# SimeonZhang/detectron2_tensorflow

Hardware: AMD Instinct MI355X
Metric: img/sec whole-node Mask R-CNN R50-FPN @1333x800 (higher is better)
Workload: dtype f32

## Files before the change

### detectron2_tensorflow_amd/csrc/conv_wgrad.hip

```cpp
#include "common.h"
#include "conv_plan.h"
#include "internal.h"

namespace d2mi {
namespace {

typedef float floatx16 __attribute__((ext_vector_type(16)));

constexpr int KP = kWgradKP;

struct WgradArgs {
  const float* x;
  const float* dy;
  float* dw;
  float* partial;
  float* dbias;
  float* pbias;
  int N, H, W, Cin, Cout, KH, KW, stride, pad, OH, OW;
  int P;
  int nCi, nCo, ntiles;
  int splits, chunks_per_split, nchunks;
  int part;
  int x_bytes, dy_bytes;
  int prio;
  int xcd;
  const uint32_t* bitmap;
};

__device__ __forceinline__ void wgrad_tile_split(const WgradArgs& a, int& tile, int& split) {
  if (!a.xcd) {
    tile = blockIdx.x;
    split = blockIdx.y;
    return;
  }
  const int nwg = gridDim.x * gridDim.y;
  const int L = blockIdx.x + blockIdx.y * gridDim.x;
  const int q = nwg / 8, r8 = nwg % 8, x8 = L % 8;
  const int l = (x8 < r8 ? x8 * (q + 1) : r8 * (q + 1) + (x8 - r8) * q) + L / 8;
  split = l / gridDim.x;
  tile = l - split * gridDim.x;
}

template <int TM, int TN>
__global__ __launch_bounds__(256, 2) void conv_wgrad_kernel(WgradArgs a) {
  constexpr int BM = 2 * TM * 32, BN = 2 * TN * 32;
  constexpr int PA = BM + 32, PB = BN + 32;
  constexpr int CA = BM / 4, CB = BN / 4;
  constexpr int RA = KP * CA / 256, RB = KP * CB / 256;
  __shared__ __attribute__((aligned(16))) float As[KP * PA];
  __shared__ __attribute__((aligned(16))) float Bs[KP * PB];

  const int tile = blockIdx.x;
  const int per_tap = a.nCi * a.nCo;
  const int tap = tile / per_tap;
  const int rem = tile - tap * per_tap;
  const int cit = rem / a.nCo, cot = rem - cit * a.nCo;
  const int kh = tap / a.KW, kw = tap - kh * a.KW;
  const int ci0 = cit * BM, co0 = cot * BN;
  const int split = blockIdx.y;
  const int c_begin = split * a.chunks_per_split;
  const int c_end = min(a.nchunks, c_begin + a.chunks_per_split);

  const int tid = threadIdx.x;
  const int lane = tid & 63, wave = tid >> 6;
  const int wr = wave >> 1, wc = wave & 1;
  const int li = lane & 31, lh = lane >> 5;

  float4 ra[RA], rb[RB];
  auto load_chunk = [&](int ch) {
    const int pbase = ch * KP;
#pragma unroll
    for (int q = 0; q < RA; ++q) {
      const int idx = tid + 256 * q;
      const int row = idx / CA, c4 = idx - row * CA;
      const int p = pbase + row;
      const int ci = ci0 + c4 * 4;
      float4 v = make_float4(0.f, 0.f, 0.f, 0.f);
      if (p < a.P && ci < a.Cin) {
        const int n = p / (a.OH * a.OW);
        const int r2 = p - n * a.OH * a.OW;
        const int oy = r2 / a.OW, ox = r2 - oy * a.OW;
        const int iy = oy * a.stride - a.pad + kh, ix = ox * a.stride - a.pad + kw;
        if (iy >= 0 && iy < a.H && ix >= 0 && ix < a.W)
          v = *reinterpret_cast<const float4*>(a.x + (((size_t)n * a.H + iy) * a.W + ix) * a.Cin +
                                               ci);
      }
      ra[q] = v;
    }
#pragma unroll
    for (int q = 0; q < RB; ++q) {
      const int idx = tid + 256 * q;
      const int row = idx / CB, c4 = idx - row * CB;
      const int p = pbase + row;
      const int co = co0 + c4 * 4;
      rb[q] = (p < a.P && co < a.Cout)
                  ? *reinterpret_cast<const float4*>(a.dy + (size_t)p * a.Cout + co)
                  : make_float4(0.f, 0.f, 0.f, 0.f);
    }
  };
  auto store_chunk = [&]() {
#pragma unroll
    for (int q = 0; q < RA; ++q) {
      const int idx = tid + 256 * q;
      const int row = idx / CA, c4 = idx - row * CA;
      *reinterpret_cast<float4*>(&As[row * PA + c4 * 4]) = ra[q];
    }
#pragma unroll
    for (int q = 0; q < RB; ++q) {
      const int idx = tid + 256 * q;
      const int row = idx / CB, c4 = idx - row * CB;
      *reinterpret_cast<float4*>(&Bs[row * PB + c4 * 4]) = rb[q];
    }
  };

  floatx16 acc[TM][TN];
#pragma unroll
  for (int i = 0; i < TM; ++i)
#pragma unroll
    for (int j = 0; j < TN; ++j)
#pragma unroll
      for (int r = 0; r < 16; ++r) acc[i][j][r] = 0.f;

  const bool do_bias = a.dbias != nullptr && tap == 0 && cit == 0;
  float bsum = 0.f;

  if (c_begin < c_end) {
    load_chunk(c_begin);
    for (int ch = c_begin; ch < c_end; ++ch) {
      store_chunk();
      __syncthreads();
      if (ch + 1 < c_end) load_chunk(ch + 1);
      if (do_bias && tid < BN) {
#pragma unroll 8
        for (int k = 0; k < KP; ++k) bsum += Bs[k * PB + tid];
      }
#pragma unroll 4
      for (int k = 0; k < KP; k += 2) {
        const float* Ar = &As[(k + lh) * PA + wr * TM * 32 + li];
        const float* Br = &Bs[(k + lh) * PB + wc * TN * 32 + li];
        float fa[TM], fb[TN];
#pragma unroll
        for (int i = 0; i < TM; ++i) fa[i] = Ar[i * 32];
#pragma unroll
        for (int j = 0; j < TN; ++j) fb[j] = Br[j * 32];
#pragma unroll
        for (int i = 0; i < TM; ++i)
#pragma unroll
          for (int j = 0; j < TN; ++j)
            acc[i][j] = __builtin_amdgcn_mfma_f32_32x32x2f32(fa[i], fb[j], acc[i][j], 0, 0, 0);
      }
      __syncthreads();
    }
  }

  if (do_bias && tid < BN && co0 + tid < a.Cout) {
    if (a.part) a.pbias[(size_t)split * a.Cout + co0 + tid] = bsum;
    else a.dbias[co0 + tid] = bsum;
  }

  const size_t wsz = (size_t)a.KH * a.KW * a.Cin * a.Cout;
  float* out = a.part ? a.partial + (size_t)split * wsz : a.dw;
#pragma unroll
  for (int j = 0; j < TN; ++j) {
    const int co = co0 + (wc * TN + j) * 32 + li;
    if (co >= a.Cout) continue;
#pragma unroll
    for (int i = 0; i < TM; ++i) {
      const int cb = ci0 + (wr * TM + i) * 32 + 4 * lh;
#pragma unroll
      for (int r = 0; r < 16; ++r) {
        const int ci = cb + (r & 3) + 8 * (r >> 2);
        if (ci < a.Cin) out[((size_t)tap * a.Cin + ci) * a.Cout + co] = acc[i][j][r];
      }
    }
  }
}

__global__ void wgrad_reduce4_kernel(const float4* __restrict__ partial, int splits, size_t total4,
                                     float4* __restrict__ dw, const float* __restrict__ pbias,
                                     int Cout, float* __restrict__ dbias, int accum) {
  const size_t n = total4 + (dbias ? (size_t)Cout : 0);
  for (size_t i = blockIdx.x * (size_t)blockDim.x + threadIdx.x; i < n;
       i += (size_t)gridDim.x * blockDim.x) {
    if (i < total4) {
      float4 s = make_float4(0.f, 0.f, 0.f, 0.f);
#pragma unroll 4
      for (int k = 0; k < splits; ++k) {
        const float4 v = partial[(size_t)k * total4 + i];
        s.x += v.x;
        s.y += v.y;
        s.z += v.z;
        s.w += v.w;
      }
      if (accum) {
        const float4 o = dw[i];
        s.x = o.x + s.x;
        s.y = o.y + s.y;
        s.z = o.z + s.z;
        s.w = o.w + s.w;
      }
      dw[i] = s;
    } else {
      const size_t c = i - total4;
      float s = 0.f;
#pragma unroll 8
      for (int k = 0; k < splits; ++k) s += pbias[(size_t)k * Cout + c];
      dbias[c] = accum ? dbias[c] + s : s;
    }
  }
}

__global__ void wgrad_reduce_kernel(const float* __restrict__ partial, int splits, size_t total,
                                    float* __restrict__ dw, const float* __restrict__ pbias,
                                    int Cout, float* __restrict__ dbias, int accum) {
  for (size_t i = blockIdx.x * (size_t)blockDim.x + threadIdx.x; i < total + Cout;
       i += (size_t)gridDim.x * blockDim.x) {
    if (i < total) {
      float s = 0.f;
#pragma unroll 4
      for (int k = 0; k < splits; ++k) s += partial[(size_t)k * total + i];
      dw[i] = accum ? dw[i] + s : s;
    } else if (dbias) {
      const size_t c = i - total;
      float s = 0.f;
#pragma unroll 8
      for (int k = 0; k < splits; ++k) s += pbias[(size_t)k * Cout + c];
      dbias[c] = accum ? dbias[c] + s : s;
    }
  }
}


typedef short bf16x8 __attribute__((ext_vector_type(8)));
constexpr int LDW = 32;

__device__ __forceinline__ int wswz(int row, int elem) {
  return row * LDW + ((((elem >> 3) ^ (row >> 2)) & 3) << 3) + (elem & 7);
}

struct FastDiv {
  uint32_t d, m, l;
};
__device__ __forceinline__ uint32_t fdiv(uint32_t n, const FastDiv& f) {
  return (__umulhi(n, f.m) + n) >> f.l;
}

template <int TM, int TN, int OCC = 2>
__global__ __launch_bounds__(256, OCC) void conv_wgrad_split_kernel(WgradArgs a, FastDiv fd_hw,
                                                                    FastDiv fd_w) {
  constexpr int BM = 2 * TM * 32, BN = 2 * TN * 32;
  constexpr int GA = BM / 4, GB = BN / 4;
  __shared__ __attribute__((aligned(16))) uint16_t As[3 * BM * LDW];
  __shared__ __attribute__((aligned(16))) uint16_t Bs[3 * BN * LDW];
  __shared__ float bred[8][BN];

  int tile, split;
  wgrad_tile_split(a, tile, split);
  const int per_tap = a.nCi * a.nCo;
  const int tap = tile / per_tap;
  const int rem = tile - tap * per_tap;
  const int cit = rem / a.nCo, cot = rem - cit * a.nCo;
  const int kh = tap / a.KW, kw = tap - kh * a.KW;
  const int ci0 = cit * BM, co0 = cot * BN;
  const int c_begin = split * a.chunks_per_split;
  const int c_end = min(a.nchunks, c_begin + a.chunks_per_split);

  const int tid = threadIdx.x;
  const int lane = tid & 63, wave = tid >> 6;
  const int wr = wave >> 1, wc = wave & 1;
  const int li = lane & 31, lh = lane >> 5;

  const bool a_on = tid < 8 * GA, b_on = tid < 8 * GB;
  const int cga = tid % GA, pga = tid / GA;
  const int cgb = tid % GB, pgb = tid / GB;
  const int ci = ci0 + 4 * cga, co = co0 + 4 * cgb;
  const bool ci_ok = a_on && ci < a.Cin, co_ok = b_on && co < a.Cout;

  const __amdgpu_buffer_rsrc_t xr = __builtin_amdgcn_make_buffer_rsrc(
      const_cast<float*>(a.x), 0, a.x_bytes, 0x00020000);
  const __amdgpu_buffer_rsrc_t yr = __builtin_amdgcn_make_buffer_rsrc(
      const_cast<float*>(a.dy), 0, a.dy_bytes, 0x00020000);
  constexpr uint32_t kOOB = 0x80000000u;

  float4 ra[4], rb[4];
  auto load_chunk = [&](int ch) {
#pragma unroll
    for (int q = 0; q < 4; ++q) {
      const int p = ch * KP + 4 * pga + q;
      const uint32_t n = fdiv((uint32_t)p, fd_hw);
      const int r2 = p - (int)n * (a.OH * a.OW);
      const int oy = (int)fdiv((uint32_t)r2, fd_w), ox = r2 - oy * a.OW;
      const int iy = oy * a.stride - a.pad + kh, ix = ox * a.stride - a.pad + kw;
      const bool ok = ci_ok & (p < a.P) & ((unsigned)iy < (unsigned)a.H) &
                      ((unsigned)ix < (unsigned)a.W);
      const uint32_t off = ok ? (uint32_t)(((((int)n * a.H + iy) * a.W + ix) * a.Cin + ci) * 4) : kOOB;
      ra[q] = __builtin_bit_cast(float4, __builtin_amdgcn_raw_buffer_load_b128(xr, off, 0, 0));
      const int pb = ch * KP + 4 * pgb + q;
      const uint32_t offb = (co_ok & (pb < a.P)) ? (uint32_t)((pb * a.Cout + co) * 4) : kOOB;
      rb[q] = __builtin_bit_cast(float4, __builtin_amdgcn_raw_buffer_load_b128(yr, offb, 0, 0));
    }
  };
  const bool do_bias = a.dbias != nullptr && tap == 0 && cit == 0;
  float bsum[4] = {0.f, 0.f, 0.f, 0.f};
  auto store_chunk = [&]() {
    if (a_on) {
      const float* f = reinterpret_cast<const float*>(ra);
#pragma unroll
      for (int j = 0; j < 4; ++j) {
        uint2 h, m, l;
        split3(make_float4(f[j], f[4 + j], f[8 + j], f[12 + j]), h, m, l);
        const int o = wswz(4 * cga + j, 4 * pga);
        *reinterpret_cast<uint2*>(&As[o]) = h;
        *reinterpret_cast<uint2*>(&As[BM * LDW + o]) = m;
        *reinterpret_cast<uint2*>(&As[2 * BM * LDW + o]) = l;
      }
    }
    if (b_on) {
      const float* f = reinterpret_cast<const float*>(rb);
#pragma unroll
      for (int j = 0; j < 4; ++j) {
        const float4 v = make_float4(f[j], f[4 + j], f[8 + j], f[12 + j]);
        if (do_bias) bsum[j] += ((v.x + v.y) + v.z) + v.w;
        uint2 h, m, l;
        split3(v, h, m, l);
        const int o = wswz(4 * cgb + j, 4 * pgb);
        *reinterpret_cast<uint2*>(&Bs[o]) = h;
        *reinterpret_cast<uint2*>(&Bs[BN * LDW + o]) = m;
        *reinterpret_cast<uint2*>(&Bs[2 * BN * LDW + o]) = l;
      }
    }
  };

  floatx16 acc[TM][TN];
#pragma unroll
  for (int i = 0; i < TM; ++i)
#pragma unroll
    for (int j = 0; j < TN; ++j)
#pragma unroll
      for (int r = 0; r < 16; ++r) acc[i][j][r] = 0.f;

  if (c_begin < c_end) {
    load_chunk(c_begin);
    for (int ch = c_begin; ch < c_end; ++ch) {
      store_chunk();
      __syncthreads();
      if (ch + 1 < c_end) load_chunk(ch + 1);
      if (a.prio) __builtin_amdgcn_s_setprio(1);
#pragma unroll
      for (int ks = 0; ks < 2; ++ks) {
        bf16x8 fa[3][TM], fb[3][TN];
#pragma unroll
        for (int pl = 0; pl < 3; ++pl) {
#pragma unroll
          for (int i = 0; i < TM; ++i)
            fa[pl][i] = *reinterpret_cast<const bf16x8*>(
                &As[pl * BM * LDW + wswz((wr * TM + i) * 32 + li, ks * 16 + lh * 8)]);
#pragma unroll
          for (int j = 0; j < TN; ++j)
            fb[pl][j] = *reinterpret_cast<const bf16x8*>(
                &Bs[pl * BN * LDW + wswz((wc * TN + j) * 32 + li, ks * 16 + lh * 8)]);
        }
        constexpr int PAi[6] = {1, 2, 0, 0, 1, 0};
        constexpr int PBi[6] = {1, 0, 2, 1, 0, 0};
#pragma unroll
        for (int t = 0; t < 6; ++t)
#pragma unroll
          for (int i = 0; i < TM; ++i)
#pragma unroll
            for (int j = 0; j < TN; ++j)
              acc[i][j] = __builtin_amdgcn_mfma_f32_32x32x16_bf16(fa[PAi[t]][i], fb[PBi[t]][j],
                                                                   acc[i][j], 0, 0, 0);
      }
      if (a.prio) __builtin_amdgcn_s_setprio(0);
      __syncthreads();
    }
  }

  if (do_bias) {
    if (b_on) {
#pragma unroll
      for (int j = 0; j < 4; ++j) bred[pgb][4 * cgb + j] = bsum[j];
    }
    __syncthreads();
    if (tid < BN && co0 + tid < a.Cout) {
      float s = 0.f;
#pragma unroll
      for (int g = 0; g < 8; ++g) s += bred[g][tid];
      if (a.part) a.pbias[(size_t)split * a.Cout + co0 + tid] = s;
      else a.dbias[co0 + tid] = s;
    }
  }

  const size_t wsz = (size_t)a.KH * a.KW * a.Cin * a.Cout;
  float* out = a.part ? a.partial + (size_t)split * wsz : a.dw;
#pragma unroll
  for (int j = 0; j < TN; ++j) {
    const int oc = co0 + (wc * TN + j) * 32 + li;
    if (oc >= a.Cout) continue;
#pragma unroll
    for (int i = 0; i < TM; ++i) {
      const int cb = ci0 + (wr * TM + i) * 32 + 4 * lh;
#pragma unroll
      for (int r = 0; r < 16; ++r) {
        const int c = cb + (r & 3) + 8 * (r >> 2);
        if (c < a.Cin) out[((size_t)tap * a.Cin + c) * a.Cout + oc] = acc[i][j][r];
      }
    }
  }
}


template <int LD, bool INC = false, bool LIST = false>
__global__ __launch_bounds__(1024, 1) void conv_wgrad_ws_kernel(WgradArgs a, FastDiv fd_hw,
                                                                FastDiv fd_w) {
  static_assert(!(LIST && INC), "the listed chunks are not consecutive");
  constexpr int TM = 2, TN = 2, BM = 256, BN = 128, S = 2;
  constexpr int GA = BM / 4, GB = BN / 4;
  constexpr int A_H = 3 * BM * LDW, B_H = 3 * BN * LDW;
  constexpr int STAGE = A_H + B_H;
  __shared__ __attribute__((aligned(16))) uint16_t smem[S * STAGE];
  __shared__ float bred[8][BN];
  __shared__ uint16_t clist[LIST ? kWgradListCap : 1];
  __shared__ int wcnt[LIST ? 17 : 1];

  int tile, split;
  wgrad_tile_split(a, tile, split);
  const int per_tap = a.nCi * a.nCo;
  const int tap = tile / per_tap;
  const int rem = tile - tap * per_tap;
  const int cit = rem / a.nCo, cot = rem - cit * a.nCo;
  const int kh = tap / a.KW, kw = tap - kh * a.KW;
  const int ci0 = cit * BM, co0 = cot * BN;
  const int c_begin = split * a.chunks_per_split;
  const int c_end = min(a.nchunks, c_begin + a.chunks_per_split);

  const int tid = threadIdx.x;
  const int lane = tid & 63;
  const int wave = __builtin_amdgcn_readfirstlane(tid >> 6);
  int nks = max(c_end - c_begin, 0);
  if constexpr (LIST) {
    const int nall = nks;
    int base = 0;
    for (int i0 = 0; i0 < nall; i0 += 1024) {
      const int i = i0 + tid;
      bool set = false;
      if (i < nall) {
        const int ch = c_begin + i;
        set = (a.bitmap[ch >> 5] >> (ch & 31)) & 1u;
      }
      const unsigned long long b = __ballot(set);
      if (lane == 0) wcnt[wave] = __popcll(b);
      __syncthreads();
      int before = base;
      for (int w = 0; w < 16; ++w) {
        const int c = wcnt[w];
        before += w < wave ? c : 0;
        base += c;
      }
      if (set) clist[before + __popcll(b & ((1ull << lane) - 1ull))] = (uint16_t)i;
      __syncthreads();
    }
    nks = __builtin_amdgcn_readfirstlane(base);
  }
  const int wr = wave >> 1, wc = wave & 1;
  const int li = lane & 31, lh = lane >> 5;
  const bool do_bias = a.dbias != nullptr && tap == 0 && cit == 0;

  floatx16 acc[TM][TN];
#pragma unroll
  for (int i = 0; i < TM; ++i)
#pragma unroll
    for (int j = 0; j < TN; ++j)
#pragma unroll
      for (int r = 0; r < 16; ++r) acc[i][j][r] = 0.f;

  if (wave >= 8) {
    const int st = tid - 512;
    const int cga = st % GA, pga = st / GA;
    const bool b_on = st >= 256;
    const int sb = st - 256;
    const int cgb = (b_on ? sb : 0) % GB, pgb = (b_on ? sb : 0) / GB;
    const int ci = ci0 + 4 * cga, co = co0 + 4 * cgb;
    const bool ci_ok = ci < a.Cin, co_ok = b_on && co < a.Cout;
    const __amdgpu_buffer_rsrc_t xr = __builtin_amdgcn_make_buffer_rsrc(
        const_cast<float*>(a.x), 0, a.x_bytes, 0x00020000);
    const __amdgpu_buffer_rsrc_t yr = __builtin_amdgcn_make_buffer_rsrc(
        const_cast<float*>(a.dy), 0, a.dy_bytes, 0x00020000);
    constexpr uint32_t kOOB = 0x80000000u;
    float4 ra[LD][4], rb[LD][4];
    const int clast = c_begin + max(nks, 1) - 1;
    int c_ch = c_begin;
    const int jlast = max(nks, 1) - 1;
    int j_ld = 0;
    const int c_first = (LIST && nks > 0) ? c_begin + clist[0] : c_begin;
    int p0 = c_first * KP + 4 * pga;
    int pb0 = c_first * KP + 4 * pgb;
    int oy0 = 0, ox0 = 0;
    if (INC) {
      const int r2 = p0 - (int)fdiv((uint32_t)p0, fd_hw) * (a.OH * a.OW);
      oy0 = (int)fdiv((uint32_t)r2, fd_w);
      ox0 = r2 - oy0 * a.OW;
    }
    const int dy32 = KP / a.OW, dx32 = KP - (KP / a.OW) * a.OW;
    const int ybase = kh - a.pad, xbase = kw - a.pad;
    const int tsh = ybase * a.W + xbase;
    const uint32_t bstride = (uint32_t)KP * (uint32_t)a.Cout * 4u;
    uint32_t boff = (uint32_t)(pb0 * a.Cout + co) * 4u;
    auto load = [&](float4 (&la)[4], float4 (&lb)[4]) {
#pragma unroll
      for (int q = 0; q < 4; ++q) {
        const int p = p0 + q;
        uint32_t off;
        if (INC) {
          int ox = ox0 + q, oy = oy0;
          const bool wrap = ox >= a.OW;
          ox = wrap ? ox - a.OW : ox;
          oy = wrap ? oy + 1 : oy;
          oy = oy >= a.OH ? oy - a.OH : oy;
          const bool ok = ci_ok & (p < a.P) & ((unsigned)(oy + ybase) < (unsigned)a.H) &
                          ((unsigned)(ox + xbase) < (unsigned)a.W);
          off = ok ? (__umul24((uint32_t)(p + tsh), (uint32_t)a.Cin) + (uint32_t)ci) * 4u : kOOB;
        } else {
          const int n = (int)fdiv((uint32_t)p, fd_hw);
          const int r2 = p - n * (a.OH * a.OW);
          const int oy = (int)fdiv((uint32_t)r2, fd_w), ox = r2 - oy * a.OW;
          const int iy = oy * a.stride - a.pad + kh, ix = ox * a.stride - a.pad + kw;
          const bool ok = ci_ok & (p < a.P) & ((unsigned)iy < (unsigned)a.H) &
                          ((unsigned)ix < (unsigned)a.W);
          off = ok ? (uint32_t)(((((int)n * a.H + iy) * a.W + ix) * a.Cin + ci) * 4) : kOOB;
        }
        la[q] = __builtin_bit_cast(float4, __builtin_amdgcn_raw_buffer_load_b128(xr, off, 0, 0));
        const uint32_t offb = (co_ok & (pb0 + q < a.P)) ? boff + (uint32_t)(q * a.Cout * 4) : kOOB;
        lb[q] = __builtin_bit_cast(float4, __builtin_amdgcn_raw_buffer_load_b128(yr, offb, 0, 0));
      }
      if constexpr (LIST) {
        if (j_ld < jlast) {
          ++j_ld;
          const int ch = c_begin + clist[j_ld];
          p0 = ch * KP + 4 * pga;
          pb0 = ch * KP + 4 * pgb;
          boff = (uint32_t)(pb0 * a.Cout + co) * 4u;
        }
      } else if (c_ch < clast) {
        ++c_ch;
        p0 += KP;
        pb0 += KP;
        boff += bstride;
        if (INC) {
          ox0 += dx32;
          oy0 += dy32;
          const bool wrap = ox0 >= a.OW;
          ox0 = wrap ? ox0 - a.OW : ox0;
          oy0 = wrap ? oy0 + 1 : oy0;
          oy0 = oy0 >= a.OH ? oy0 - a.OH : oy0;
        }
      }
    };
    float bsum[4] = {0.f, 0.f, 0.f, 0.f};
    auto write = [&](int buf, const float4 (&la)[4], const float4 (&lb)[4]) {
      uint16_t* As = smem + buf * STAGE;
      uint16_t* Bs = As + A_H;
      const float* f = reinterpret_cast<const float*>(la);
#pragma unroll
      for (int j = 0; j < 4; ++j) {
        uint2 h, m, l;
        split3(make_float4(f[j], f[4 + j], f[8 + j], f[12 + j]), h, m, l);
        const int o = wswz(4 * cga + j, 4 * pga);
        *reinterpret_cast<uint2*>(&As[o]) = h;
        *reinterpret_cast<uint2*>(&As[BM * LDW + o]) = m;
        *reinterpret_cast<uint2*>(&As[2 * BM * LDW + o]) = l;
      }
      if (b_on) {
        const float* g = reinterpret_cast<const float*>(lb);
#pragma unroll
        for (int j = 0; j < 4; ++j) {
          const float4 v = make_float4(g[j], g[4 + j], g[8 + j], g[12 + j]);
          if (do_bias) bsum[j] += ((v.x + v.y) + v.z) + v.w;
          uint2 h, m, l;
          split3(v, h, m, l);
          const int o = wswz(4 * cgb + j, 4 * pgb);
          *reinterpret_cast<uint2*>(&Bs[o]) = h;
          *reinterpret_cast<uint2*>(&Bs[BN * LDW + o]) = m;
          *reinterpret_cast<uint2*>(&Bs[2 * BN * LDW + o]) = l;
        }
      }
    };
#pragma unroll
    for (int j = 0; j < LD; ++j) load(ra[j], rb[j]);
    if (nks > 0) write(0, ra[0], rb[0]);
    load(ra[0], rb[0]);
    __syncthreads();
    int u0 = 0;
    for (; u0 + LD <= nks; u0 += LD) {
#pragma unroll
      for (int j = 0; j < LD; ++j) {
        const int v = u0 + j + 1;
        const int set = (j + 1) % LD;
        if (v < nks) write(v & 1, ra[set], rb[set]);
        load(ra[set], rb[set]);
        __syncthreads();
      }
    }
#pragma unroll
    for (int j = 0; j < LD - 1; ++j) {
      if (u0 + j < nks) {
        const int v = u0 + j + 1;
        const int set = (j + 1) % LD;
        if (v < nks) write(v & 1, ra[set], rb[set]);
        __syncthreads();
      }
    }
    if (do_bias && b_on) {
#pragma unroll
      for (int j = 0; j < 4; ++j) bred[pgb][4 * cgb + j] = bsum[j];
    }
  } else {
    bf16x8 fa[3][TM], fb[3][TN];
    auto ld1 = [&](const uint16_t* As, const uint16_t* Bs, int pa, int pb, int ks) {
#pragma unroll
      for (int i = 0; i < TM; ++i)
        fa[pa][i] = *reinterpret_cast<const bf16x8*>(
            &As[pa * BM * LDW + wswz((wr * TM + i) * 32 + li, ks * 16 + lh * 8)]);
#pragma unroll
      for (int j = 0; j < TN; ++j)
        fb[pb][j] = *reinterpret_cast<const bf16x8*>(
            &Bs[pb * BN * LDW + wswz((wc * TN + j) * 32 + li, ks * 16 + lh * 8)]);
    };
    auto mm1 = [&](int pa, int pb) {
#pragma unroll
      for (int i = 0; i < TM; ++i)
#pragma unroll
        for (int j = 0; j < TN; ++j)
          acc[i][j] =
              __builtin_amdgcn_mfma_f32_32x32x16_bf16(fa[pa][i], fb[pb][j], acc[i][j], 0, 0, 0);
    };
    auto step16 = [&](const uint16_t* As, const uint16_t* Bs, int ks) {
      ld1(As, Bs, 1, 1, ks);
      __builtin_amdgcn_sched_barrier(0);
      ld1(As, Bs, 2, 0, ks);
      mm1(1, 1);
      __builtin_amdgcn_sched_barrier(0);
      ld1(As, Bs, 0, 2, ks);
      mm1(2, 0);
      __builtin_amdgcn_sched_barrier(0);
      mm1(0, 2);
      mm1(0, 1);
      mm1(1, 0);
      mm1(0, 0);
    };
    __syncthreads();
    for (int u = 0; u < nks; ++u) {
      const uint16_t* As = smem + (u & 1) * STAGE;
      const uint16_t* Bs = As + A_H;
      if (a.prio) __builtin_amdgcn_s_setprio(1);
      step16(As, Bs, 0);
      step16(As, Bs, 1);
      if (a.prio) __builtin_amdgcn_s_setprio(0);
      __builtin_amdgcn_sched_barrier(0);
      __syncthreads();
    }
  }
  if (do_bias) {
    __syncthreads();
    if (tid < BN && co0 + tid < a.Cout) {
      float s = 0.f;
#pragma unroll
      for (int g = 0; g < 8; ++g) s += bred[g][tid];
      if (a.part) a.pbias[(size_t)split * a.Cout + co0 + tid] = s;
      else a.dbias[co0 + tid] = s;
    }
  }
  if (wave >= 8) return;
  const size_t wsz = (size_t)a.KH * a.KW * a.Cin * a.Cout;
  float* out = a.part ? a.partial + (size_t)split * wsz : a.dw;
#pragma unroll
  for (int j = 0; j < TN; ++j) {
    const int oc = co0 + (wc * TN + j) * 32 + li;
    if (oc >= a.Cout) continue;
#pragma unroll
    for (int i = 0; i < TM; ++i) {
      const int cb = ci0 + (wr * TM + i) * 32 + 4 * lh;
#pragma unroll
      for (int r = 0; r < 16; ++r) {
        const int c = cb + (r & 3) + 8 * (r >> 2);
        if (c < a.Cin) out[((size_t)tap * a.Cin + c) * a.Cout + oc] = acc[i][j][r];
      }
    }
  }
}

FastDiv make_fastdiv(uint32_t d) {
  FastDiv f;
  f.d = d;
  uint32_t l = 0;
  while ((1ull << l) < d) ++l;
  f.l = l;
  f.m = (uint32_t)((((1ull << 32) * ((1ull << l) - d)) / d) + 1);
  return f;
}

}
}

using namespace d2mi;

extern "C" size_t d2mi_conv2d_wgrad_workspace_size(int N, int H, int W, int Cin, int Cout, int KH,
                                                   int KW, int stride, int pad_beg, int pad_end) {
  if (N <= 0 || H <= 0 || W <= 0 || Cin <= 0 || Cout <= 0 || KH <= 0 || KW <= 0 || stride <= 0)
    return 0;
  const ConvShape s = {N, H, W, Cin, Cout, KH, KW, stride, pad_beg, pad_end};
  WgradPlan split, f32;
  if (plan_wgrad(s, kPlanSplit3, kOpAllAligned | kOpWorkspace, SIZE_MAX, &split) ||
      plan_wgrad(s, 0, kOpAllAligned | kOpWorkspace, SIZE_MAX, &f32))
    return 0;
  return std::max(split.ws_bytes, f32.ws_bytes);
}

static int wgrad_plan_checked(int N, int H, int W, int Cin, int Cout, int KH, int KW, int stride,
                              int pad_beg, int pad_end, int flags, int operands,
                              size_t workspace_bytes, WgradPlan* p) {
  D2MI_REQUIRE((flags & ~12) == 0,
               "wgrad flags: bit2 = split-bf16 products, bit3 = accumulate into dw / dbias");
  D2MI_REQUIRE(N > 0 && H > 0 && W > 0 && Cin > 0 && Cout > 0 && KH > 0 && KW > 0 && stride > 0,
               "bad conv shape");
  D2MI_REQUIRE(Cin % 4 == 0 && Cout % 4 == 0, "Cin and Cout must be multiples of 4 (%d, %d)",
               Cin, Cout);
  int OH, OW;
  D2MI_REQUIRE(conv_dims(H, W, KH, KW, stride, pad_beg, pad_end, OH, OW) == 0,
               "conv output is empty");
  D2MI_REQUIRE((long long)N * OH * OW < (1LL << 31), "too many pixels");
  if (flags & kPlanSplit3)
    D2MI_REQUIRE((int64_t)N * H * W * Cin * 4 < (1ll << 31) &&
                     (int64_t)N * OH * OW * Cout * 4 < (1ll << 31),
                 "split wgrad: x and dy must each be < 2 GiB");
  plan_wgrad({N, H, W, Cin, Cout, KH, KW, stride, pad_beg, pad_end}, flags, operands,
             workspace_bytes, p);
  if (flags & kPlanAccum)
    D2MI_REQUIRE((operands & kOpWorkspace) && workspace_bytes >= p->ws_bytes,
                 "accumulating wgrad: workspace must hold %d slab(s)", p->splits);
  return 0;
}

extern "C" int d2mi_conv2d_wgrad_plan(int N, int H, int W, int Cin, int Cout, int KH, int KW,
                                      int stride, int pad_beg, int pad_end, int flags,
                                      int operands, size_t workspace_bytes, int32_t* out,
                                      int out_len) {
  D2MI_REQUIRE((operands & ~127) == 0, "wgrad plan: unknown operand bits");
  WgradPlan p;
  if (wgrad_plan_checked(N, H, W, Cin, Cout, KH, KW, stride, pad_beg, pad_end, flags, operands,
                         workspace_bytes, &p))
    return -1;
  const int32_t v[] = {p.kernel, p.TM, p.TN, p.BM, p.BN, p.nCi, p.nCo, p.ntiles, p.nchunks,
                       p.splits, p.chunks_per_split, p.part, p.reduce, p.reduce_grid,
                       (int32_t)(p.ws_bytes & 0x7fffffff), (int32_t)(p.ws_bytes >> 31)};
  return emit_plan(v, (int)(sizeof(v) / sizeof(v[0])), out, out_len);
}

static int wgrad_launch(const float* x, const float* dy, float* dw_hwio, float* dbias, int N,
                        int H, int W, int Cin, int Cout, int KH, int KW, int stride, int pad_beg,
                        int pad_end, int flags, const uint32_t* bitmap, void* workspace,
                        size_t workspace_bytes, void* stream) {
  auto al16 = [](const void* q) { return ((uintptr_t)q & 15) == 0; };
  WgradPlan p;
  if (wgrad_plan_checked(N, H, W, Cin, Cout, KH, KW, stride, pad_beg, pad_end, flags,
                         (al16(dw_hwio) ? kOpAligned : 0) | (workspace ? kOpWorkspace : 0) |
                             (al16(workspace) ? kOpWsAligned : 0),
                         workspace_bytes, &p))
    return -1;
  D2MI_REQUIRE(al16(x) && al16(dy), "x and dy must be 16-byte aligned");
  WgradSpace sp = {};
  if (p.part) {
    Workspace carve(workspace, workspace_bytes);
    sp.lay(carve, p.splits, (size_t)KH * KW * Cin * Cout, Cout);
  }
  WgradArgs a = {};
  a.prio = tuning(kTuneWgradPrio);
  a.xcd = tuning(kTuneWgradXCD) > 0 ? 1 : 0;
  a.x = x;
  a.dy = dy;
  a.dw = dw_hwio;
  a.dbias = dbias;
  a.N = N;
  a.H = H;
  a.W = W;
  a.Cin = Cin;
  a.Cout = Cout;
  a.KH = KH;
  a.KW = KW;
  a.stride = stride;
  a.pad = pad_beg;
  a.OH = p.OH;
  a.OW = p.OW;
  a.P = N * a.OH * a.OW;
  a.nCi = p.nCi;
  a.nCo = p.nCo;
  a.ntiles = p.ntiles;
  a.splits = p.splits;
  a.chunks_per_split = p.chunks_per_split;
  a.nchunks = p.nchunks;
  a.part = p.part;
  a.partial = sp.dw;
  a.pbias = sp.dbias;
  hipStream_t st = as_stream(stream);
  const dim3 grid(p.ntiles, p.splits);
  if (p.kernel != kWgradF32) {
    a.x_bytes = (int)((int64_t)N * H * W * Cin * 4);
    a.dy_bytes = (int)((int64_t)a.P * Cout * 4);
  }
  const FastDiv fhw = make_fastdiv((uint32_t)(a.OH * a.OW)), fw = make_fastdiv((uint32_t)a.OW);
  const int tm = p.TM, tn = p.TN;
  const bool listed = bitmap != nullptr && p.chunks_per_split <= kWgradListCap &&
                      (p.kernel == kWgradWSInc || p.kernel == kWgradWS);
  a.bitmap = listed ? bitmap : nullptr;
  if (listed)
    hipLaunchKernelGGL((conv_wgrad_ws_kernel<1, false, true>), grid, dim3(1024), 0, st, a, fhw, fw);
  else if (p.kernel == kWgradWSInc)
    hipLaunchKernelGGL((conv_wgrad_ws_kernel<1, true>), grid, dim3(1024), 0, st, a, fhw, fw);
  else if (p.kernel == kWgradWS)
    hipLaunchKernelGGL((conv_wgrad_ws_kernel<1>), grid, dim3(1024), 0, st, a, fhw, fw);
  else if (p.kernel == kWgradSplitOcc3)
    hipLaunchKernelGGL((conv_wgrad_split_kernel<2, 2, 3>), grid, dim3(256), 0, st, a, fhw, fw);
  else if (p.kernel == kWgradSplit && tm == 2 && tn == 2)
    hipLaunchKernelGGL((conv_wgrad_split_kernel<2, 2>), grid, dim3(256), 0, st, a, fhw, fw);
  else if (p.kernel == kWgradSplit && tm == 2)
    hipLaunchKernelGGL((conv_wgrad_split_kernel<2, 1>), grid, dim3(256), 0, st, a, fhw, fw);
  else if (p.kernel == kWgradSplit && tn == 2)
    hipLaunchKernelGGL((conv_wgrad_split_kernel<1, 2>), grid, dim3(256), 0, st, a, fhw, fw);
  else if (p.kernel == kWgradSplit)
    hipLaunchKernelGGL((conv_wgrad_split_kernel<1, 1>), grid, dim3(256), 0, st, a, fhw, fw);
  else if (tm == 2 && tn == 2)
    hipLaunchKernelGGL((conv_wgrad_kernel<2, 2>), grid, dim3(256), 0, st, a);
  else if (tm == 2)
    hipLaunchKernelGGL((conv_wgrad_kernel<2, 1>), grid, dim3(256), 0, st, a);
  else if (tn == 2)
    hipLaunchKernelGGL((conv_wgrad_kernel<1, 2>), grid, dim3(256), 0, st, a);
  else
    hipLaunchKernelGGL((conv_wgrad_kernel<1, 1>), grid, dim3(256), 0, st, a);
  D2MI_LAUNCH_CHECK();
  if (p.reduce == kReduceNone) return listed ? 1 : 0;
  const size_t total = (size_t)KH * KW * Cin * Cout;
  const int accum = (flags & kPlanAccum) != 0;
  if (p.reduce == kReduceFloat4)
    hipLaunchKernelGGL(wgrad_reduce4_kernel, dim3(p.reduce_grid), dim3(256), 0, st,
                       reinterpret_cast<const float4*>(a.partial), a.splits, total / 4,
                       reinterpret_cast<float4*>(dw_hwio), a.pbias, Cout, dbias, accum);
  else
    hipLaunchKernelGGL(wgrad_reduce_kernel, dim3(p.reduce_grid), dim3(256), 0, st, a.partial,
                       a.splits, total, dw_hwio, a.pbias, Cout, dbias, accum);
  D2MI_LAUNCH_CHECK();
  return listed ? 1 : 0;
}

extern "C" int d2mi_conv2d_wgrad_ex(const float* x, const float* dy, float* dw_hwio,
                                    float* dbias, int N, int H, int W, int Cin, int Cout, int KH,
                                    int KW, int stride, int pad_beg, int pad_end, int flags,
                                    void* workspace, size_t workspace_bytes, void* stream) {
  return wgrad_launch(x, dy, dw_hwio, dbias, N, H, W, Cin, Cout, KH, KW, stride, pad_beg, pad_end,
                      flags, nullptr, workspace, workspace_bytes, stream);
}

extern "C" int d2mi_conv2d_wgrad_rows(const float* x, const float* dy, float* dw_hwio,
                                      float* dbias, int N, int H, int W, int Cin, int Cout, int KH,
                                      int KW, int stride, int pad_beg, int pad_end, int flags,
                                      const void* census, size_t census_bytes, void* workspace,
                                      size_t workspace_bytes, void* stream) {
  int OH, OW;
  D2MI_REQUIRE(N > 0 && H > 0 && W > 0 && KH > 0 && KW > 0 && stride > 0 &&
                   conv_dims(H, W, KH, KW, stride, pad_beg, pad_end, OH, OW) == 0 &&
                   (long long)N * OH * OW < (1LL << 31),
               "bad conv shape");
  RowCensusSpace cs;
  Workspace carve(const_cast<void*>(census), census_bytes);
  cs.lay(carve, N * OH * OW, 0);
  D2MI_REQUIRE(census != nullptr && carve.ok(), "row census workspace too small (%zu < %zu)",
               census_bytes, carve.off);
  D2MI_REQUIRE(((uintptr_t)census & 3) == 0, "the row census must be 4-byte aligned");
  return wgrad_launch(x, dy, dw_hwio, dbias, N, H, W, Cin, Cout, KH, KW, stride, pad_beg, pad_end,
                      flags, cs.bitmap, workspace, workspace_bytes, stream);
}


extern "C" int d2mi_conv2d_wgrad(const float* x, const float* dy, float* dw_hwio, float* dbias,
                                 int N, int H, int W, int Cin, int Cout, int KH, int KW,
                                 int stride, int pad_beg, int pad_end, void* workspace,
                                 size_t workspace_bytes, void* stream) {
  return d2mi_conv2d_wgrad_ex(x, dy, dw_hwio, dbias, N, H, W, Cin, Cout, KH, KW, stride,
                              pad_beg, pad_end, 0, workspace, workspace_bytes, stream);
}
```

Measured before the change: 113.2.

## Add two-stage LDS pipeline with deep register prefetch to split wgrad kernel

Adds a variant of the split-K weight-gradient kernel with two LDS stages and a three-chunk register prefetch ring. The bf16 split-and-store and the global loads are interleaved with the MFMA sequence using sched_group_barrier hints, which removes one barrier per chunk. This variant is used only when the grid fits within one wave of CUs (occupancy 1). Larger grids keep the original single-stage kernel. The cost is more LDS and registers per block, plus tail-handling logic that is harder to get right.

```diff
diff --git a/detectron2_tensorflow_amd/csrc/conv_wgrad.hip b/detectron2_tensorflow_amd/csrc/conv_wgrad.hip
--- a/detectron2_tensorflow_amd/csrc/conv_wgrad.hip
+++ b/detectron2_tensorflow_amd/csrc/conv_wgrad.hip
@@ -245,13 +245,15 @@
   return (__umulhi(n, f.m) + n) >> f.l;
 }
 
-template <int TM, int TN, int OCC = 2>
+template <int TM, int TN, int OCC = 2, int LD = 1, int ST = 1>
 __global__ __launch_bounds__(256, OCC) void conv_wgrad_split_kernel(WgradArgs a, FastDiv fd_hw,
                                                                     FastDiv fd_w) {
+  static_assert(ST == 1 || ST == 2, "one or two LDS stages");
   constexpr int BM = 2 * TM * 32, BN = 2 * TN * 32;
   constexpr int GA = BM / 4, GB = BN / 4;
-  __shared__ __attribute__((aligned(16))) uint16_t As[3 * BM * LDW];
-  __shared__ __attribute__((aligned(16))) uint16_t Bs[3 * BN * LDW];
+  constexpr int A_H = 3 * BM * LDW, B_H = 3 * BN * LDW;
+  constexpr int STAGE = A_H + B_H;
+  __shared__ __attribute__((aligned(16))) uint16_t smem[ST * STAGE];
   __shared__ float bred[8][BN];
 
   int tile, split;
@@ -270,7 +272,8 @@
   const int wr = wave >> 1, wc = wave & 1;
   const int li = lane & 31, lh = lane >> 5;
 
-  const bool a_on = tid < 8 * GA, b_on = tid < 8 * GB;
+  const bool a_on = (ST == 2 && 8 * GA >= 256) || tid < 8 * GA;
+  const bool b_on = (ST == 2 && 8 * GB >= 256) || tid < 8 * GB;
   const int cga = tid % GA, pga = tid / GA;
   const int cgb = tid % GB, pgb = tid / GB;
   const int ci = ci0 + 4 * cga, co = co0 + 4 * cgb;
@@ -282,31 +285,34 @@
       const_cast<float*>(a.dy), 0, a.dy_bytes, 0x00020000);
   constexpr uint32_t kOOB = 0x80000000u;
 
-  float4 ra[4], rb[4];
-  auto load_chunk = [&](int ch) {
-#pragma unroll
-    for (int q = 0; q < 4; ++q) {
-      const int p = ch * KP + 4 * pga + q;
-      const uint32_t n = fdiv((uint32_t)p, fd_hw);
-      const int r2 = p - (int)n * (a.OH * a.OW);
-      const int oy = (int)fdiv((uint32_t)r2, fd_w), ox = r2 - oy * a.OW;
-      const int iy = oy * a.stride - a.pad + kh, ix = ox * a.stride - a.pad + kw;
-      const bool ok = ci_ok & (p < a.P) & ((unsigned)iy < (unsigned)a.H) &
-                      ((unsigned)ix < (unsigned)a.W);
-      const uint32_t off = ok ? (uint32_t)(((((int)n * a.H + iy) * a.W + ix) * a.Cin + ci) * 4) : kOOB;
-      ra[q] = __builtin_bit_cast(float4, __builtin_amdgcn_raw_buffer_load_b128(xr, off, 0, 0));
-      const int pb = ch * KP + 4 * pgb + q;
-      const uint32_t offb = (co_ok & (pb < a.P)) ? (uint32_t)((pb * a.Cout + co) * 4) : kOOB;
-      rb[q] = __builtin_bit_cast(float4, __builtin_amdgcn_raw_buffer_load_b128(yr, offb, 0, 0));
-    }
+  float4 ra[LD][4], rb[LD][4];
+  auto load_q = [&](float4 (&la)[4], float4 (&lb)[4], int ch, int q) {
+    const bool in = (LD == 1 && ST == 1) || ch < c_end;
+    const int p = ch * KP + 4 * pga + q;
+    const uint32_t n = fdiv((uint32_t)p, fd_hw);
+    const int r2 = p - (int)n * (a.OH * a.OW);
+    const int oy = (int)fdiv((uint32_t)r2, fd_w), ox = r2 - oy * a.OW;
+    const int iy = oy * a.stride - a.pad + kh, ix = ox * a.stride - a.pad + kw;
+    const bool ok = in & ci_ok & (p < a.P) & ((unsigned)iy < (unsigned)a.H) &
+                    ((unsigned)ix < (unsigned)a.W);
+    const uint32_t off = ok ? (uint32_t)(((((int)n * a.H + iy) * a.W + ix) * a.Cin + ci) * 4) : kOOB;
+    la[q] = __builtin_bit_cast(float4, __builtin_amdgcn_raw_buffer_load_b128(xr, off, 0, 0));
+    const int pb = ch * KP + 4 * pgb + q;
+    const uint32_t offb = (in & co_ok & (pb < a.P)) ? (uint32_t)((pb * a.Cout + co) * 4) : kOOB;
+    lb[q] = __builtin_bit_cast(float4, __builtin_amdgcn_raw_buffer_load_b128(yr, offb, 0, 0));
+  };
+  auto load = [&](float4 (&la)[4], float4 (&lb)[4], int ch) {
+#pragma unroll
+    for (int q = 0; q < 4; ++q) load_q(la, lb, ch, q);
   };
   const bool do_bias = a.dbias != nullptr && tap == 0 && cit == 0;
   float bsum[4] = {0.f, 0.f, 0.f, 0.f};
-  auto store_chunk = [&]() {
-    if (a_on) {
-      const float* f = reinterpret_cast<const float*>(ra);
-#pragma unroll
-      for (int j = 0; j < 4; ++j) {
+  auto write_unit = [&](uint16_t* As, const float4 (&la)[4], const float4 (&lb)[4], int k) {
+    uint16_t* Bs = As + A_H;
+    if (k < 4) {
+      if (a_on) {
+        const int j = k;
+        const float* f = reinterpret_cast<const float*>(la);
         uint2 h, m, l;
         split3(make_float4(f[j], f[4 + j], f[8 + j], f[12 + j]), h, m, l);
         const int o = wswz(4 * cga + j, 4 * pga);
@@ -314,21 +320,22 @@
         *reinterpret_cast<uint2*>(&As[BM * LDW + o]) = m;
         *reinterpret_cast<uint2*>(&As[2 * BM * LDW + o]) = l;
       }
-    }
-    if (b_on) {
-      const float* f = reinterpret_cast<const float*>(rb);
-#pragma unroll
-      for (int j = 0; j < 4; ++j) {
-        const float4 v = make_float4(f[j], f[4 + j], f[8 + j], f[12 + j]);
-        if (do_bias) bsum[j] += ((v.x + v.y) + v.z) + v.w;
-        uint2 h, m, l;
-        split3(v, h, m, l);
-        const int o = wswz(4 * cgb + j, 4 * pgb);
-        *reinterpret_cast<uint2*>(&Bs[o]) = h;
-        *reinterpret_cast<uint2*>(&Bs[BN * LDW + o]) = m;
-        *reinterpret_cast<uint2*>(&Bs[2 * BN * LDW + o]) = l;
-      }
-    }
+    } else if (b_on) {
+      const int j = k - 4;
+      const float* f = reinterpret_cast<const float*>(lb);
+      const float4 v = make_float4(f[j], f[4 + j], f[8 + j], f[12 + j]);
+      if (do_bias) bsum[j] += ((v.x + v.y) + v.z) + v.w;
+      uint2 h, m, l;
+      split3(v, h, m, l);
+      const int o = wswz(4 * cgb + j, 4 * pgb);
+      *reinterpret_cast<uint2*>(&Bs[o]) = h;
+      *reinterpret_cast<uint2*>(&Bs[BN * LDW + o]) = m;
+      *reinterpret_cast<uint2*>(&Bs[2 * BN * LDW + o]) = l;
+    }
+  };
+  auto write = [&](uint16_t* As, const float4 (&la)[4], const float4 (&lb)[4]) {
+#pragma unroll
+    for (int k = 0; k < 8; ++k) write_unit(As, la, lb, k);
   };
 
   floatx16 acc[TM][TN];
@@ -339,40 +346,103 @@
 #pragma unroll
       for (int r = 0; r < 16; ++r) acc[i][j][r] = 0.f;
 
-  if (c_begin < c_end) {
-    load_chunk(c_begin);
-    for (int ch = c_begin; ch < c_end; ++ch) {
-      store_chunk();
+  bf16x8 fa[3][TM], fb[3][TN];
+  auto ld1 = [&](const uint16_t* As, int pa, int pb, int ks) {
+    const uint16_t* Bs = As + A_H;
+#pragma unroll
+    for (int i = 0; i < TM; ++i)
+      fa[pa][i] = *reinterpret_cast<const bf16x8*>(
+          &As[pa * BM * LDW + wswz((wr * TM + i) * 32 + li, ks * 16 + lh * 8)]);
+#pragma unroll
+    for (int j = 0; j < TN; ++j)
+      fb[pb][j] = *reinterpret_cast<const bf16x8*>(
+          &Bs[pb * BN * LDW + wswz((wc * TN + j) * 32 + li, ks * 16 + lh * 8)]);
+  };
+  auto mm1 = [&](int pa, int pb) {
+#pragma unroll
+    for (int i = 0; i < TM; ++i)
+#pragma unroll
+      for (int j = 0; j < TN; ++j)
+        acc[i][j] =
+            __builtin_amdgcn_mfma_f32_32x32x16_bf16(fa[pa][i], fb[pb][j], acc[i][j], 0, 0, 0);
+  };
+  constexpr int PAi[6] = {1, 2, 0, 0, 1, 0};
+  constexpr int PBi[6] = {1, 0, 2, 1, 0, 0};
+  auto compute = [&](const uint16_t* As) {
+#pragma unroll
+    for (int ks = 0; ks < 2; ++ks) {
+#pragma unroll
+      for (int pl = 0; pl < 3; ++pl) ld1(As, pl, pl, ks);
+#pragma unroll
+      for (int t = 0; t < 6; ++t) mm1(PAi[t], PBi[t]);
+    }
+  };
+  auto seg_end = [&](bool staging) {
+    if constexpr (TM * TN == 4) {
+#pragma unroll
+      for (int i = 0; i < 4; ++i) {
+        __builtin_amdgcn_sched_group_barrier(0x008, 1, 0);
+        __builtin_amdgcn_sched_group_barrier(0x002, 7, 0);
+        if (staging) {
+          if (i < 3) __builtin_amdgcn_sched_group_barrier(0x200, 1, 0);
+        } else if (i >= 2) {
+          __builtin_amdgcn_sched_group_barrier(0x020, 1, 0);
+        }
+      }
+    }
+    __builtin_amdgcn_sched_barrier(0);
+  };
+  auto step2 = [&](int u, float4 (&la)[4], float4 (&lb)[4]) {
+    const uint16_t* As = smem + (u & 1) * STAGE;
+    uint16_t* Aw = smem + ((u + 1) & 1) * STAGE;
+    const int chl = c_begin + u + 1 + LD;
+    ld1(As, 1, 1, 0);
+    __builtin_amdgcn_sched_barrier(0);
+#pragma unroll
+    for (int ks = 0; ks < 2; ++ks) {
+#pragma unroll
+      for (int t = 0; t < 6; ++t) {
+        if (t == 0) ld1(As, 2, 0, ks);
+        if (t == 1) ld1(As, 0, 2, ks);
+        if (t == 5 && ks == 0) ld1(As, 1, 1, 1);
+        mm1(PAi[t], PBi[t]);
+        const int g = ks * 6 + t;
+        if (g < 8) write_unit(Aw, la, lb, g);
+        else load_q(la, lb, chl, g - 8);
+        seg_end(g < 8);
+      }
+    }
+    __syncthreads();
+  };
+
+  const int nch = c_end - c_begin;
+  if (nch > 0) {
+#pragma unroll
+    for (int j = 0; j < LD; ++j) load(ra[j], rb[j], c_begin + j);
+    if constexpr (ST == 2) {
+      write(smem, ra[0], rb[0]);
+      load(ra[0], rb[0], c_begin + LD);
       __syncthreads();
-      if (ch + 1 < c_end) load_chunk(ch + 1);
-      if (a.prio) __builtin_amdgcn_s_setprio(1);
-#pragma unroll
-      for (int ks = 0; ks < 2; ++ks) {
-        bf16x8 fa[3][TM], fb[3][TN];
-#pragma unroll
-        for (int pl = 0; pl < 3; ++pl) {
-#pragma unroll
-          for (int i = 0; i < TM; ++i)
-            fa[pl][i] = *reinterpret_cast<const bf16x8*>(
-                &As[pl * BM * LDW + wswz((wr * TM + i) * 32 + li, ks * 16 + lh * 8)]);
-#pragma unroll
-          for (int j = 0; j < TN; ++j)
-            fb[pl][j] = *reinterpret_cast<const bf16x8*>(
-                &Bs[pl * BN * LDW + wswz((wc * TN + j) * 32 + li, ks * 16 + lh * 8)]);
-        }
-        constexpr int PAi[6] = {1, 2, 0, 0, 1, 0};
-        constexpr int PBi[6] = {1, 0, 2, 1, 0, 0};
-#pragma unroll
-        for (int t = 0; t < 6; ++t)
-#pragma unroll
-          for (int i = 0; i < TM; ++i)
-#pragma unroll
-            for (int j = 0; j < TN; ++j)
-              acc[i][j] = __builtin_amdgcn_mfma_f32_32x32x16_bf16(fa[PAi[t]][i], fb[PBi[t]][j],
-                                                                   acc[i][j], 0, 0, 0);
-      }
-      if (a.prio) __builtin_amdgcn_s_setprio(0);
-      __syncthreads();
+      int u0 = 0;
+      for (; u0 + LD < nch; u0 += LD) {
+#pragma unroll
+        for (int j = 0; j < LD; ++j) step2(u0 + j, ra[(j + 1) % LD], rb[(j + 1) % LD]);
+      }
+#pragma unroll
+      for (int j = 0; j < LD - 1; ++j)
+        if (u0 + j + 1 < nch) step2(u0 + j, ra[(j + 1) % LD], rb[(j + 1) % LD]);
+      compute(smem + ((nch - 1) & 1) * STAGE);
+    } else {
+      static_assert(ST == 2 || LD == 1, "the one-stage form is the plain double buffer");
+      for (int u = 0; u < nch; ++u) {
+        write(smem, ra[0], rb[0]);
+        __syncthreads();
+        if (u + 1 < nch) load(ra[0], rb[0], c_begin + u + 1);
+        if (a.prio) __builtin_amdgcn_s_setprio(1);
+        compute(smem);
+        if (a.prio) __builtin_amdgcn_s_setprio(0);
+        __syncthreads();
+      }
     }
   }
 
@@ -754,6 +824,30 @@
                        p.splits, p.chunks_per_split, p.part, p.reduce, p.reduce_grid,
                        (int32_t)(p.ws_bytes & 0x7fffffff), (int32_t)(p.ws_bytes >> 31)};
   return emit_plan(v, (int)(sizeof(v) / sizeof(v[0])), out, out_len);
+}
+
+static int wgrad_device_cus() {
+  static int cus = 0;
+  if (cus == 0) {
+    int dev = 0, c = 0;
+    if (hipGetDevice(&dev) != hipSuccess ||
+        hipDeviceGetAttribute(&c, hipDeviceAttributeMultiprocessorCount, dev) != hipSuccess ||
+        c <= 0)
+      c = 256;
+    cus = c;
+  }
+  return cus;
+}
+
+constexpr int kSplitLD = 3;
+template <int TM, int TN>
+static void launch_split(dim3 grid, hipStream_t st, const WgradArgs& a, FastDiv fhw, FastDiv fw) {
+  if ((int)(grid.x * grid.y) <= wgrad_device_cus())
+    hipLaunchKernelGGL((conv_wgrad_split_kernel<TM, TN, 1, kSplitLD, 2>), grid,
+                       dim3(256), 0, st, a, fhw, fw);
+  else
+    hipLaunchKernelGGL((conv_wgrad_split_kernel<TM, TN, 2, 1, 1>), grid, dim3(256), 0, st, a, fhw,
+                       fw);
 }
 
 static int wgrad_launch(const float* x, const float* dy, float* dw_hwio, float* dbias, int N,
@@ -821,13 +915,13 @@
   else if (p.kernel == kWgradSplitOcc3)
     hipLaunchKernelGGL((conv_wgrad_split_kernel<2, 2, 3>), grid, dim3(256), 0, st, a, fhw, fw);
   else if (p.kernel == kWgradSplit && tm == 2 && tn == 2)
-    hipLaunchKernelGGL((conv_wgrad_split_kernel<2, 2>), grid, dim3(256), 0, st, a, fhw, fw);
+    launch_split<2, 2>(grid, st, a, fhw, fw);
   else if (p.kernel == kWgradSplit && tm == 2)
-    hipLaunchKernelGGL((conv_wgrad_split_kernel<2, 1>), grid, dim3(256), 0, st, a, fhw, fw);
+    launch_split<2, 1>(grid, st, a, fhw, fw);
   else if (p.kernel == kWgradSplit && tn == 2)
-    hipLaunchKernelGGL((conv_wgrad_split_kernel<1, 2>), grid, dim3(256), 0, st, a, fhw, fw);
+    launch_split<1, 2>(grid, st, a, fhw, fw);
   else if (p.kernel == kWgradSplit)
-    hipLaunchKernelGGL((conv_wgrad_split_kernel<1, 1>), grid, dim3(256), 0, st, a, fhw, fw);
+    launch_split<1, 1>(grid, st, a, fhw, fw);
   else if (tm == 2 && tn == 2)
     hipLaunchKernelGGL((conv_wgrad_kernel<2, 2>), grid, dim3(256), 0, st, a);
   else if (tm == 2)
```

Result: no change. 114.0, median of 6 (+0.7%).
